# cheukwaylee/ORB_SLAM2_detailed_comments

Hardware: AMD Instinct MI355X
Metric: frames/sec ORB extract+match (1000 kp, 640x480) (higher is better)
Workload: dtype u8; 1 GPU; synthetic 640x480 mono stream, nFeatures=1000, 8 levels, scale 1.2, FAST 20/7, extract+match(t vs t-1), batch 1024 frames/GPU resident in HBM, 1 pipelines/GPU; parallelism=single GPU

## Files before the change

orb_slam2_detailed_comments_amd/csrc/orbx_api.cpp:

```cpp
#include <hip/hip_runtime.h>
#include <dlfcn.h>
#include <cstdio>
#include <cstdlib>
#include <cstring>
#include <string>
#include <vector>
#include <algorithm>
#include <cmath>
#include "orbx_internal.h"
#include "orbx_launch.h"
#include "orbx_gate.h"

static thread_local std::string g_last_error;
#define ORBX_RGBD_INPLACE_DEFAULT true

static orbx_status fail(orbx_status s, const std::string &msg) {
    g_last_error = msg;
    return s;
}
#define HIPCHK(expr)                                                                              \
    do {                                                                                          \
        hipError_t _e = (expr);                                                                   \
        if (_e != hipSuccess)                                                                     \
            return fail(ORBX_HIP_ERROR, std::string(#expr) + ": " + hipGetErrorString(_e));      \
// ... 13 lines not shown
    hipEvent_t ev_fork = nullptr, ev_join = nullptr;
    hipEvent_t ev_stereo = nullptr;
    int fork_level = 0;
    int fork_group = 0;
    int pipeline = 2;
    bool pipe_head = true;
    bool fast_room = false;
    hipEvent_t ev_pipe[ORBX_PIPE_MAX] = {};
    uint8_t *d_pyr = nullptr, *d_blur = nullptr;
    OrbxCell *d_cells = nullptr;
    OrbxFastGroup *d_groups = nullptr;
    bool resize_legacy = false;
    int match_kernel = 0;
    int fast_stop = 0;
    int fast_lcap = 640;
    OrbxTap *d_taps = nullptr;
    uint2 *d_dense = nullptr;
    int *d_cand_count = nullptr, *d_lvl_count = nullptr, *d_status = nullptr;
    uint32_t *d_lvl_kp = nullptr;
    float *d_lvl_angle = nullptr;
    uint16_t *d_knode = nullptr;
    int max_cw = 0, max_ch = 0, ncap = 0, lds_keys = 0, lds_keys_few = 0;
    uint8_t *st_in[2] = {nullptr, nullptr}; size_t d_in_bytes = 0;
    orbx_keypoint *st_kps[2] = {nullptr, nullptr}; uint8_t *st_desc[2] = {nullptr, nullptr}; int *st_cnt[2] = {nullptr, nullptr};
    int out_cap = 0, stage_chunk = 0;
    int *pin_stat = nullptr; size_t pin_stat_ints = 0;
    hipStream_t s_in = nullptr;
    hipEvent_t ev_in[2] = {nullptr, nullptr}, ev_done[2] = {nullptr, nullptr}, ev_out[2] = {nullptr, nullptr};
    uint8_t *st_dep[2] = {nullptr, nullptr}; size_t dep_bytes = 0;
    uint8_t *st_rg[2] = {nullptr, nullptr}; size_t rg_bytes = 0;
    int last_batch = 0;
// ... 87 lines not shown
    if (h->pending.empty()) return;
    hipStreamSynchronize(h->stream);
    for (auto &pp : h->pending) {
        float ms = 0;
        if (hipEventElapsedTime(&ms, pp.a, pp.b) == hipSuccess) { h->ms[pp.kid] += ms; h->launches[pp.kid]++; }
        h->pool.push_back(pp.a); h->pool.push_back(pp.b);
    }
    h->pending.clear();
}

static orbx_status pin_reserve(orbx_handle *h, size_t bytes);

static void free_geometry_buffers(orbx_handle *h) {
    hipFree(h->d_groups); h->d_groups = nullptr;
    hipFree(h->d_pyr); hipFree(h->d_blur); hipFree(h->d_cells); hipFree(h->d_taps);
    hipFree(h->d_dense); h->d_dense = nullptr;
    hipFree(h->d_cand_count); hipFree(h->d_lvl_count); hipFree(h->d_status); hipFree(h->d_lvl_kp);
    hipFree(h->d_lvl_angle); hipFree(h->d_knode);
    h->d_pyr = h->d_blur = nullptr; h->d_cells = nullptr; h->d_taps = nullptr;
    h->d_cand_count = h->d_lvl_count = h->d_status = nullptr; h->d_lvl_kp = nullptr; h->d_lvl_angle = nullptr;
    h->d_knode = nullptr;
    h->configured = false;
}

static orbx_status configure(orbx_handle *h, int width, int height) {
    if (h->configured && h->geom.width == width && h->geom.height == height) return ORBX_OK;
    if (h->host_only) return fail(ORBX_NO_DEVICE, "host-only handle (device = -2) cannot extract");
    HIPCHK(hipSetDevice(h->dev));
    if (h->configured) {
        HIPCHK(hipStreamSynchronize(h->stream));
// ... 40 lines not shown
            const size_t budget = (size_t)(160 * 1024) / wg - 512;
            return budget <= node_part ? 0 : std::min<size_t>({(budget - node_part) / 6, (size_t)4096, (size_t)g.max_cand_cap});
        };
        size_t keys_few = 0;
        for (int wg = 4; wg >= 2 && keys == 0; --wg)
            if (fit_at(wg) >= want) { keys = std::max<size_t>(want, 1024); keys_few = fit_at(wg); }
        h->lds_keys_few = (int)keys_few;
        if (keys == 0 && fit_at(2) >= 1024) keys = fit_at(2);
        if (keys == 0) keys = fit_at(1);
        if (const char *e = getenv("ORBX_QT_LDS_KEYS")) keys = std::min<size_t>((size_t)std::max(atoi(e), 0), std::min<size_t>(8192, (160 * 1024 - node_part) / 6));
        h->lds_keys = (int)keys;
        if (getenv("ORBX_QT_LDS_KEYS") || h->lds_keys_few < h->lds_keys) h->lds_keys_few = h->lds_keys;
    }
    HIPCHK(orbx_quadtree_prepare(orbx_quadtree_smem(h->ncap, std::max(h->lds_keys, h->lds_keys_few))));
    if (const char *e = getenv("ORBX_RESIZE_IMPL")) h->resize_legacy = strcmp(e, "legacy") == 0;
#ifdef ORBX_TIMING_KNOBS
    if (const char *e = getenv("ORBX_FAST_STOP")) h->fast_stop = atoi(e);
#endif
    if (const char *e = getenv("ORBX_FAST_LCAP")) h->fast_lcap = std::max(64, atoi(e));
    const OrbxGeom &hg = h->geom;
    hipStream_t s = h->stream;
    h->fork_level = 0;
    if (const char *e = getenv("ORBX_FORK_LEVEL")) h->fork_level = std::min(std::max(atoi(e), 0), NL - 1);
    h->fork_group = 0;
    if (h->fork_level > 0) {
        while (h->fork_group < (int)hg.fast_groups.size() && hg.cells[(size_t)hg.fast_groups[(size_t)h->fork_group].cell0].level < h->fork_level)
            ++h->fork_group;
        if (h->fork_group == 0 || h->fork_group >= (int)hg.fast_groups.size()) h->fork_level = 0;
    }
    if (const char *e = getenv("ORBX_PIPELINE")) h->pipeline = std::min(std::max(atoi(e), 0), ORBX_PIPE_MAX);
// ... 7 lines not shown
        ORBX_TRY(hipMalloc(&h->d_cells, std::max<size_t>(1, hg.cells.size()) * sizeof(OrbxCell)));
        ORBX_TRY(hipMalloc(&h->d_taps, std::max<size_t>(1, hg.taps.size()) * sizeof(OrbxTap)));
        ORBX_TRY(hipMalloc(&h->d_dense, (size_t)B * hg.cand_total * sizeof(uint2)));
        ORBX_TRY(hipMalloc(&h->d_knode, (size_t)B * hg.cand_total * sizeof(uint16_t)));
        ORBX_TRY(hipMalloc(&h->d_cand_count, (size_t)B * NL * sizeof(int)));
        ORBX_TRY(hipMalloc(&h->d_lvl_count, (size_t)B * NL * sizeof(int)));
        ORBX_TRY(hipMalloc(&h->d_status, (size_t)B * sizeof(int)));
        ORBX_TRY(hipMalloc(&h->d_lvl_kp, (size_t)B * hg.kp_total * sizeof(uint32_t)));
        ORBX_TRY(hipMalloc(&h->d_lvl_angle, (size_t)B * hg.kp_total * sizeof(float)));
        ORBX_TRY(hipMalloc(&h->d_groups, std::max<size_t>(1, hg.fast_groups.size()) * sizeof(OrbxFastGroup)));
        if (!hg.cells.empty()) {
            ORBX_TRY(hipMemcpyAsync(h->d_cells, hg.cells.data(), hg.cells.size() * sizeof(OrbxCell), hipMemcpyHostToDevice, s));
            ORBX_TRY(hipMemcpyAsync(h->d_groups, hg.fast_groups.data(), hg.fast_groups.size() * sizeof(OrbxFastGroup),
                                    hipMemcpyHostToDevice, s));
        }
        if (!hg.taps.empty())
            ORBX_TRY(hipMemcpyAsync(h->d_taps, hg.taps.data(), hg.taps.size() * sizeof(OrbxTap), hipMemcpyHostToDevice, s));
        ORBX_TRY(hipMemsetAsync(h->d_pyr, 0, (size_t)B * hg.pyr_bytes + 256, s));
        ORBX_TRY(hipMemsetAsync(h->d_lvl_count, 0, (size_t)B * NL * sizeof(int), s));
        ORBX_TRY(hipMemsetAsync(h->d_cand_count, 0, (size_t)B * NL * sizeof(int), s));
#undef ORBX_TRY
        return hipSuccess;
    };
    const hipError_t se = setup();
    if (se != hipSuccess) {
        hipStreamSynchronize(s);
        free_geometry_buffers(h);
        return fail(ORBX_HIP_ERROR, std::string("configure: ") + hipGetErrorString(se));
    }
    h->configured = true;
    h->last_batch = 0;
    return ORBX_OK;
// ... 143 lines not shown
    const DGeom &g = h->dg;
    hipStream_t s = h->stream;
    const int NL = g.nlevels;
    if (h->d_rect && (h->rect_w != W || h->rect_h != H))
        return fail(ORBX_BAD_ARGUMENT, "rectification maps were set for another image size (raw and rectified size must agree)");
    const int ngroups = (int)h->geom.fast_groups.size();
    auto pyramid = [&](hipStream_t st, int f0, int b, int l_end) {
        const uint8_t *im = d_imgs + (int64_t)f0 * frame_stride;
        uint8_t *pyr = h->d_pyr + (size_t)f0 * h->geom.pyr_bytes;
        int32_t *stp = d_status + f0;
        int *cc = h->d_cand_count + (size_t)f0 * NL;
        { ProfScope ps(h, ORBX_K_PYR_L0, st);
          if (h->d_rect) {
              orbx_launch_pyr_l0_remap(st, g, b, im, W, H, stride, frame_stride, pyr, h->d_rect, stp, cc);
          } else if (h->input_format == ORBX_FMT_GRAY8) {
              orbx_launch_pyr_l0(st, g, b, im, W, H, stride, frame_stride, pyr, stp, cc);
          } else {
              const int nch = (h->input_format == ORBX_FMT_RGB8 || h->input_format == ORBX_FMT_BGR8) ? 3 : 4;
              const bool rgb = h->input_format == ORBX_FMT_RGB8 || h->input_format == ORBX_FMT_RGBA8;
              orbx_launch_pyr_l0_color(st, g, b, im, W, H, stride, frame_stride, pyr, nch, rgb ? 0 : 2, rgb ? 2 : 0, stp, cc);
          } }
        for (int l = 1; l < l_end; ++l) {
            ProfScope ps(h, ORBX_K_PYR_RESIZE, st);
            orbx_launch_pyr_resize(st, g, b, l, h->d_taps, pyr, h->geom.lv[l].narrow_taps && !h->resize_legacy);
        }
    };
    auto fast = [&](hipStream_t st, int f0, int b, int g0, int ng, int lds_floor) {
        ProfScope ps(h, ORBX_K_FAST, st);
        orbx_launch_fast_rows(st, g, b, h->d_cells, h->d_groups + g0, ng, h->d_pyr + (size_t)f0 * h->geom.pyr_bytes,
                              h->d_dense + (size_t)f0 * g.cand_total, h->d_cand_count + (size_t)f0 * NL, d_status + f0, h->max_ch,
                              h->fast_lcap, h->fast_stop, lds_floor);
    };
    auto finish = [&](int f0, int b) {
        { ProfScope ps(h, ORBX_K_QUADTREE);
          orbx_launch_quadtree(s, g, b, h->d_dense + (size_t)f0 * g.cand_total, h->d_cand_count + (size_t)f0 * NL,
                               h->d_lvl_kp + (size_t)f0 * g.kp_total, h->d_lvl_count + (size_t)f0 * NL, d_status + f0,
                               h->d_knode + (size_t)f0 * g.cand_total, h->ncap, (long long)b * NL >= 1024 ? h->lds_keys : h->lds_keys_few, 0, NL); }
        { ProfScope ps(h, ORBX_K_DESC);
          orbx_launch_describe(s, g, b, h->d_pyr + (size_t)f0 * h->geom.pyr_bytes, h->d_lvl_kp + (size_t)f0 * g.kp_total,
// ... 27 lines not shown
            finish(off[k], off[k + 1] - off[k]);
        }
        hipError_t e = hipGetLastError();
        if (e != hipSuccess) { hipStreamSynchronize(s2); return fail(ORBX_HIP_ERROR, std::string("kernel launch: ") + hipGetErrorString(e)); }
        h->last_batch = B;
        return ORBX_OK;
    }
    const bool fork = h->fork_level > 0 && (long long)B * ngroups >= 16384;
    pyramid(s, 0, B, fork ? h->fork_level : NL);
    if (fork) {
        hipStream_t s2 = h->side_stream;
        if (hipEventRecord(h->ev_fork, s) != hipSuccess || hipStreamWaitEvent(s2, h->ev_fork, 0) != hipSuccess)
            return fail(ORBX_HIP_ERROR, "fork event");
        for (int l = h->fork_level; l < NL; ++l) {
            ProfScope ps(h, ORBX_K_PYR_RESIZE, s2);
            orbx_launch_pyr_resize(s2, g, B, l, h->d_taps, h->d_pyr, h->geom.lv[l].narrow_taps && !h->resize_legacy);
        }
        fast(s2, 0, B, h->fork_group, ngroups - h->fork_group, 0);
        fast(s, 0, B, 0, h->fork_group, 0);
        if (hipEventRecord(h->ev_join, s2) != hipSuccess || hipStreamWaitEvent(s, h->ev_join, 0) != hipSuccess)
            { hipStreamSynchronize(s2); return fail(ORBX_HIP_ERROR, "join event"); }
    } else {
        fast(s, 0, B, 0, ngroups, 0);
    }
    finish(0, B);
    hipError_t e = hipGetLastError();
    if (e != hipSuccess) return fail(ORBX_HIP_ERROR, std::string("kernel launch: ") + hipGetErrorString(e));
    h->last_batch = B;
    return ORBX_OK;
}

// ... 1464 lines not shown
```

orb_slam2_detailed_comments_amd/csrc/orbx_geometry.cpp:

```cpp
#include "orbx_internal.h"
#include <cmath>
#include <algorithm>

static inline int cv_round_f(float v) { return (int)lrintf(v); }
static inline int cv_round_d(double v) { return (int)lrint(v); }
static inline int cv_floor_f(float v) { int i = (int)v; return i - (i > v); }
static inline int cv_ceil_f(float v) { int i = (int)v; return i + (i < v); }
static inline int16_t sat16(int v) { return (int16_t)std::min(32767, std::max(-32768, v)); }
static inline int reflect101(int i, int n) {
    if (n == 1) return 0;
    while (i < 0 || i >= n) i = i < 0 ? -i : 2 * (n - 1) - i;
    return i;
}

void orbx_build_tables(const orbx_params &p, OrbxTables &t) {
    const int L = p.nlevels;
    const double sf = (double)p.scale_factor;
    t.scale[0] = 1.0f;
    t.sigma2[0] = 1.0f;
    for (int i = 1; i < L; ++i) {
        t.scale[i] = (float)((double)t.scale[i - 1] * sf);
        t.sigma2[i] = t.scale[i] * t.scale[i];
    }
    for (int i = 0; i < L; ++i) {
// ... 141 lines not shown
        }
    }
    for (size_t i = 0; i < g.cells.size();) {
        const OrbxCell &a = g.cells[i];
        OrbxFastGroup grp;
        grp.cell0 = (int32_t)i; grp.ncell = 1;
        if (i + 1 < g.cells.size()) {
            const OrbxCell &b = g.cells[i + 1];
            const bool adjacent = b.level == a.level && b.y0 == a.y0 && b.ch == a.ch && b.x0 == a.x0 + a.cw - 6 &&
                                  b.idx_in_level == a.idx_in_level + 1;
            if (adjacent && (a.cw - 6) + (b.cw - 6) <= 64 + ORBX_FAST_XCOLS) grp.ncell = 2;
        }
        g.fast_groups.push_back(grp);
        i += (size_t)grp.ncell;
    }
    g.pyr_bytes = off;
    g.cand_total = cand_off;
    g.kp_total = kp_off;
    return ORBX_OK;
}
```

orb_slam2_detailed_comments_amd/csrc/orbx_internal.h:

```cpp
#pragma once
#include <cstdint>
#include <vector>
#include "../../include/orbx.h"

#define ORBX_MAX_LEVELS 16
#define ORBX_EDGE 19
#define ORBX_HALF_PATCH 15
#define ORBX_PATCH 31
#define ORBX_NPATCH 749

struct OrbxCell {
    int16_t x0, y0, cw, ch;
    int16_t offx, offy;
    int16_t level;
    int16_t idx_in_level;
    int32_t slot_begin;
    int32_t slot_cap;
};

#define ORBX_FAST_XCOLS 2
struct OrbxFastGroup {
    int32_t cell0;
    int32_t ncell;
};
#define ORBX_LDS_PER_CU (160 * 1024)
#define ORBX_FAST_PIPE_WAVES 16
#define ORBX_PIPE_MAX 8
#define ORBX_PIPE_MIN_FRAMES 256

struct OrbxTap {
    int16_t s0, s1;
    int16_t a0, a1;
};

struct OrbxLevelGeom {
    int sw, sh;
    int pw, ph, pitch;
    int64_t off;
    int ncols, nrows, wcell, hcell;
    int cell_begin, cell_count;
    int qt_w, qt_h;
    int nini;
    float hx;
    int nfeat;
    int kp_cap;
    int kp_begin;
    int cand_cap;
    int64_t cand_begin;
    int tapx_begin, tapy_begin;
    bool narrow_taps;
    float scale;
    float size;
};

struct OrbxGeom {
    int width = 0, height = 0, nlevels = 0;
    OrbxLevelGeom lv[ORBX_MAX_LEVELS];
    std::vector<OrbxCell> cells;
    std::vector<OrbxFastGroup> fast_groups;
    std::vector<OrbxTap> taps;
    int64_t pyr_bytes = 0;
    int64_t cand_total = 0;
    int kp_total = 0;
    int node_cap = 0;
    int max_cand_cap = 0;
};

struct OrbxTables {
    float scale[ORBX_MAX_LEVELS], inv_scale[ORBX_MAX_LEVELS], sigma2[ORBX_MAX_LEVELS], inv_sigma2[ORBX_MAX_LEVELS];
    int nfeat[ORBX_MAX_LEVELS];
    int umax[ORBX_HALF_PATCH + 1];
};

void orbx_build_tables(const orbx_params &p, OrbxTables &t);
orbx_status orbx_build_geometry(const orbx_params &p, const OrbxTables &t, int width, int height, OrbxGeom &g,
// ... 2 lines not shown
```

orb_slam2_detailed_comments_amd/csrc/orbx_kernels.hip:

```cpp
#include "orbx_device.h"
#include "../../include/orbx_pattern_data.h"

#define L0_ROWS 8
#ifndef L0_FF
#define L0_FF 1
#endif
#ifndef RR_FF
#define RR_FF 1
#endif
#ifndef QT_FF
#define QT_FF 1
#endif
__global__ __launch_bounds__(256) void k_pyr_l0(DGeom g, const uint8_t *__restrict__ imgs, int W, int H, int stride,
                                                long long frame_stride, uint8_t *__restrict__ pyr, int xe,
                                                int *__restrict__ status, int *__restrict__ cand_cursor) {
    const DLevel &L = g.lv[0];
#if L0_FF
    const int f = blockIdx.x, bx = blockIdx.y, by = blockIdx.z, nbx = gridDim.y;
#else
    const int f = blockIdx.z, bx = blockIdx.x, by = blockIdx.y, nbx = gridDim.x;
#endif
    if (bx == 0 && by == 0 && threadIdx.y == 0) {
        if (threadIdx.x == 0) status[f] = 0;
        if ((int)threadIdx.x < g.nlevels) cand_cursor[f * g.nlevels + threadIdx.x] = 0;
// ... 26 lines not shown
#pragma unroll
        for (int r = 0; r < L0_ROWS; ++r) {
            const int Y = Y0 + r;
            if (Y >= L.ph) break;
            const uint8_t *src = img + (long long)orbx_reflect101(Y - ORBX_EDGE, H) * stride;
            uint32_t w = 0;
#pragma unroll
            for (int i = 0; i < 4; ++i) {
                const int x = X + i;
                const uint32_t p = x < L.pw ? src[orbx_reflect101(x - ORBX_EDGE, W)] : 0u;
                w |= p << (8 * i);
            }
            *(uint32_t *)(dst + (long long)Y * L.pitch + X) = w;
        }
    }
}

__global__ __launch_bounds__(256) void k_pyr_l0_color(DGeom g, const uint8_t *__restrict__ imgs, int W, int H, int stride,
                                                      long long frame_stride, uint8_t *__restrict__ pyr, int nch,
                                                      int r_off, int b_off, int *__restrict__ status, int *__restrict__ cand_cursor) {
    const DLevel &L = g.lv[0];
    const int X = (blockIdx.x * 64 + threadIdx.x) * 4;
    const int Y = blockIdx.y * 4 + threadIdx.y;
    const int f = blockIdx.z;
    if (blockIdx.x == 0 && blockIdx.y == 0 && threadIdx.y == 0) {
        if (threadIdx.x == 0) status[f] = 0;
        if ((int)threadIdx.x < g.nlevels) cand_cursor[f * g.nlevels + threadIdx.x] = 0;
    }
    if (X >= L.pw || Y >= L.ph) return;
    const uint8_t *src = imgs + (long long)f * frame_stride + (long long)orbx_reflect101(Y - ORBX_EDGE, H) * stride;
// ... 39 lines not shown
            const uint8_t *r0 = src + (long long)iy * stride + ix, *r1 = r0 + stride;
            const uint32_t p00 = (x0 && y0) ? r0[0] : 0u, p01 = (x1 && y0) ? r0[1] : 0u, p10 = (x0 && y1) ? r1[0] : 0u,
                           p11 = (x1 && y1) ? r1[1] : 0u;
            const uint32_t acc = __umul24((32u - fx) * (32u - fy) * 32u, p00) + __umul24(fx * (32u - fy) * 32u, p01) +
                                 __umul24((32u - fx) * fy * 32u, p10) + __umul24(fx * fy * 32u, p11);
            p = (acc + (1u << 14)) >> 15;
        }
        v |= p << (8 * i);
    }
    *(uint32_t *)(pyr + (long long)f * g.pyr_bytes + L.off + (long long)Y * L.pitch + X) = v;
}

struct __attribute__((packed, aligned(1))) orbx_uint2_u { uint32_t x, y; };
struct __attribute__((packed, aligned(1))) orbx_uint3_u { uint32_t x, y, z; };
__device__ __forceinline__ uint2 orbx_load8(const void *p) { const orbx_uint2_u v = *(const orbx_uint2_u *)p; return make_uint2(v.x, v.y); }
struct __attribute__((aligned(4))) orbx_uint3_a { uint32_t x, y, z; };
typedef unsigned short orbx_v2u16 __attribute__((ext_vector_type(2)));
__device__ __forceinline__ uint32_t orbx_udot2(uint32_t a, uint32_t b) {
    return __builtin_amdgcn_udot2(__builtin_bit_cast(orbx_v2u16, a), __builtin_bit_cast(orbx_v2u16, b), 0u, false);
}
#define RS_ROWS 2
__global__ __launch_bounds__(256) void k_pyr_resize(DGeom g, int level, const OrbxTap *__restrict__ taps,
                                                    uint8_t *__restrict__ pyr) {
    const DLevel &L = g.lv[level];
    const DLevel &S = g.lv[level - 1];
    const int X = (blockIdx.x * 64 + threadIdx.x) * 4;
    const int Y0 = (blockIdx.y * 4 + threadIdx.y) * RS_ROWS;
    const int f = blockIdx.z;
    if (X >= L.pw || Y0 >= L.ph) return;
    uint8_t *base = pyr + (long long)f * g.pyr_bytes;
    OrbxTap tx[4];
    int smin = 0x7fff, smax = 0;
#pragma unroll
    for (int i = 0; i < 4; ++i) {
// ... 75 lines not shown
                const int T1 = r1[tx[i].s0] * tx[i].a0 + r1[tx[i].s1] * tx[i].a1;
                const uint32_t p = (uint32_t)((((((b0 & 0xfff) * ((T0 >> 4) & 0xffff))) >> 16) + ((((b1 & 0xfff) * ((T1 >> 4) & 0xffff))) >> 16) + 2) >> 2) & 0xffu;
                v |= p << (8 * i);
            }
        }
        *(uint32_t *)(base + L.off + (long long)Y * L.pitch + X) = v;
    }
}

#ifndef RR_REVERSE
#define RR_REVERSE 1
#endif
#ifndef RR_WPB
#define RR_WPB 1
#endif
__global__ __launch_bounds__(64 * RR_WPB) void k_pyr_resize_rows(DGeom g, int level, const OrbxTap *__restrict__ taps,
                                                         uint8_t *__restrict__ pyr, int rpw) {
    const DLevel &L = g.lv[level];
    const DLevel &S = g.lv[level - 1];
    const int lane = threadIdx.x;
#if RR_FF
    const int f = blockIdx.x, bx = blockIdx.y;
    const int by = (RR_REVERSE && (level & 1)) ? (int)gridDim.z - 1 - (int)blockIdx.z : (int)blockIdx.z;
#else
    const int f = blockIdx.z, bx = blockIdx.x, by = blockIdx.y;
#endif
    const int X = (bx * 64 + lane) * 4;
    const int y_begin = __builtin_amdgcn_readfirstlane((by * RR_WPB + threadIdx.y) * rpw);
    if (y_begin >= L.ph) return;
    const int y_end = min(y_begin + rpw, L.ph);
    const bool on = X < L.pw;
    uint8_t *base = pyr + (long long)f * g.pyr_bytes;
// ... 6 lines not shown
        const uint2 *tq = (const uint2 *)taps + L.tapx;
        uint2 t[4];
#pragma unroll
        for (int i = 0; i < 4; ++i) t[i] = tq[min(X + i, L.pw - 1)];
#pragma unroll
        for (int i = 0; i < 4; ++i) smin = min(smin, (int)(t[i].x & 0xffffu));
#pragma unroll
        for (int i = 0; i < 4; ++i) {
            const uint32_t d = (t[i].x & 0xffffu) - (uint32_t)smin;
            sel[i] = d | (0x0cu << 8) | ((d + 1u) << 16) | (0x0cu << 24);
            wgt[i] = t[i].y;
        }
    }
    const uint32_t sh = (uint32_t)(smin & 3);
    const uint32_t lsrc = (uint32_t)(smin & ~3);
    const uint2 *ty = (const uint2 *)taps + L.tapy;
#ifndef RR_R
#define RR_R 2
#endif
#define RR_H(dst, v)                                                                                                     \
    {                                                                                                                   \
        const uint32_t lo_ = __builtin_amdgcn_alignbyte((v).y, (v).x, sh), hi_ = __builtin_amdgcn_alignbyte((v).z, (v).y, sh); \
        _Pragma("unroll") for (int i = 0; i < 4; ++i)                                                                   \
            dst[i] = orbx_udot2(__builtin_amdgcn_perm(hi_, lo_, sel[i]), wgt[i]) >> 4;                                  \
    }
#define RR_V(out, h0, h1, w0, w1)                                                                                       \
    {                                                                                                                   \
        out = 0;                                                                                                        \
        _Pragma("unroll") for (int i = 0; i < 4; ++i)                                                                   \
            out |= (((__umul24(w0, h0[i]) >> 16) + (__umul24(w1, h1[i]) >> 16) + 2u) >> 2) << (8 * i);                  \
    }
    uint2 t[RR_R];
    orbx_uint3_a u[RR_R], w[RR_R];
    int pid = -1;
    uint32_t hb[2][4] = {{0, 0, 0, 0}, {0, 0, 0, 0}};
#pragma unroll
    for (int r = 0; r < RR_R; ++r) {
        t[r] = ty[min(y_begin + r, L.ph - 1)];
        u[r].x = u[r].y = u[r].z = 0;
        if (r == 0 || (int)(t[r].x & 0xffffu) != (int)(t[r - 1].x >> 16)) u[r] = *(const orbx_uint3_a *)(src + (uint32_t)((t[r].x & 0xffffu) * (uint32_t)S.pitch + lsrc));
        w[r] = *(const orbx_uint3_a *)(src + (uint32_t)((t[r].x >> 16) * (uint32_t)S.pitch + lsrc));
    }
    for (int Y = y_begin; Y < y_end; Y += RR_R) {
        uint2 ct[RR_R];
        orbx_uint3_a cu[RR_R], cw[RR_R];
#pragma unroll
        for (int r = 0; r < RR_R; ++r) { ct[r] = t[r]; cu[r] = u[r]; cw[r] = w[r]; }
        if (Y + RR_R < y_end) {
            int last = (int)(ct[RR_R - 1].x >> 16);
#pragma unroll
            for (int r = 0; r < RR_R; ++r) {
                t[r] = ty[min(Y + RR_R + r, L.ph - 1)];
                const int s0 = (int)(t[r].x & 0xffffu), s1 = (int)(t[r].x >> 16);
                if (s0 != last) u[r] = *(const orbx_uint3_a *)(src + (uint32_t)((uint32_t)s0 * (uint32_t)S.pitch + lsrc));
                w[r] = *(const orbx_uint3_a *)(src + (uint32_t)((uint32_t)s1 * (uint32_t)S.pitch + lsrc));
                last = s1;
            }
        }
#pragma unroll
        for (int r = 0; r < RR_R; ++r) {
            uint32_t (&h0)[4] = hb[r & 1], (&h1)[4] = hb[(r & 1) ^ 1];
            const int s0 = (int)(ct[r].x & 0xffffu);
            if (s0 != pid) RR_H(h0, cu[r])
            RR_H(h1, cw[r])
            uint32_t v;
            RR_V(v, h0, h1, ct[r].y & 0xfffu, (ct[r].y >> 16) & 0xfffu)
            pid = (int)(ct[r].x >> 16);
            if (on && Y + r < y_end) *(uint32_t *)(dst + (uint32_t)((uint32_t)(Y + r) * (uint32_t)L.pitch + ldst)) = v;
        }
    }
#undef RR_H
#undef RR_V
}

__device__ __forceinline__ bool orbx_arc9(uint32_t mask16) {
    uint32_t m = mask16 | (mask16 << 16);
    uint32_t a = m & (m >> 1);
    a &= a >> 2;
    a &= a >> 4;
    a &= m >> 8;
    return (a & 0xffffu) != 0;
}

__device__ __forceinline__ unsigned long long orbx_ballot(bool p) { return __builtin_amdgcn_ballot_w64(p); }
__device__ __forceinline__ int orbx_wave_rank(unsigned long long bal) {
// ... 2413 lines not shown
            for (int sl = 0; sl < 16; ++sl) {
                const int k = 16 * (lane >> 4) + sl, i = k - (16 * j + (lane & 15));
                if (i >= 0 && i <= 6) bb[j][lane][sl >> 2] |= (uint32_t)K7[i] << (8 * (sl & 3));
            }
    return hipMemcpyToSymbol(HIP_SYMBOL(c_blur_b), bb, sizeof(bb));
}

size_t orbx_quadtree_smem(int ncap, int lds_keys) {
    return 128 + (size_t)ncap * (8 * 4 + 16 + 8 + 6 * 4) + 16 + (size_t)lds_keys * 6 + 16;
}

void orbx_launch_clear(hipStream_t s, int *a, int na, int *b, int nb, int *c, int nc) {
    const int n = na > nb ? (na > nc ? na : nc) : (nb > nc ? nb : nc);
    hipLaunchKernelGGL(k_clear, dim3((n + 255) / 256), dim3(256), 0, s, a, na, b, nb, c, nc);
}
void orbx_launch_pyr_l0(hipStream_t s, const DGeom &g, int B, const uint8_t *imgs, int W, int H, int stride,
                        long long frame_stride, uint8_t *pyr, int *status, int *cand_cursor) {
    const DLevel &L = g.lv[0];
    int xe = 32;
    while (xe + 1 <= W) xe += 16;
    const int icols = (xe - 32 + 1023) / 1024;
#if L0_FF
    dim3 grid(B, icols + 1, (L.ph + 4 * L0_ROWS - 1) / (4 * L0_ROWS));
#else
    dim3 grid(icols + 1, (L.ph + 4 * L0_ROWS - 1) / (4 * L0_ROWS), B);
#endif
    hipLaunchKernelGGL(k_pyr_l0, grid, dim3(64, 4), 0, s, g, imgs, W, H, stride, frame_stride, pyr, xe, status, cand_cursor);
}
void orbx_launch_pyr_l0_color(hipStream_t s, const DGeom &g, int B, const uint8_t *imgs, int W, int H, int stride,
                              long long frame_stride, uint8_t *pyr, int nch, int r_off, int b_off, int *status, int *cand_cursor) {
    const DLevel &L = g.lv[0];
    dim3 grid((L.pw + 255) / 256, (L.ph + 3) / 4, B);
    hipLaunchKernelGGL(k_pyr_l0_color, grid, dim3(64, 4), 0, s, g, imgs, W, H, stride, frame_stride, pyr, nch, r_off, b_off, status, cand_cursor);
}
void orbx_launch_pyr_l0_remap(hipStream_t s, const DGeom &g, int B, const uint8_t *imgs, int W, int H, int stride,
                              long long frame_stride, uint8_t *pyr, const uint2 *rect, int *status, int *cand_cursor) {
    const DLevel &L = g.lv[0];
    dim3 grid((L.pw + 255) / 256, (L.ph + 3) / 4, B);
    hipLaunchKernelGGL(k_pyr_l0_remap, grid, dim3(64, 4), 0, s, g, imgs, W, H, stride, frame_stride, pyr, rect, status, cand_cursor);
}
void orbx_launch_pyr_resize(hipStream_t s, const DGeom &g, int B, int level, const OrbxTap *taps, uint8_t *pyr, bool narrow) {
    const DLevel &L = g.lv[level];
    if (narrow) {
        int rpw = 16;
        while (rpw > 2 && (long long)((L.pw + 255) / 256) * ((L.ph + rpw - 1) / rpw) * B < 4096) rpw >>= 1;
#if RR_FF
        dim3 grid(B, (L.pw + 255) / 256, (L.ph + RR_WPB * rpw - 1) / (RR_WPB * rpw));
#else
        dim3 grid((L.pw + 255) / 256, (L.ph + RR_WPB * rpw - 1) / (RR_WPB * rpw), B);
#endif
        hipLaunchKernelGGL(k_pyr_resize_rows, grid, dim3(64, RR_WPB), 0, s, g, level, taps, pyr, rpw);
        return;
    }
    dim3 grid((L.pw + 255) / 256, (L.ph + 4 * RS_ROWS - 1) / (4 * RS_ROWS), B);
    hipLaunchKernelGGL(k_pyr_resize, grid, dim3(64, 4), 0, s, g, level, taps, pyr);
}
void orbx_launch_fast_rows(hipStream_t s, const DGeom &g, int B, const OrbxCell *cells, const OrbxFastGroup *groups,
                           int ngroups, const uint8_t *pyr, uint2 *cand, int *cand_cursor, int *status, int max_ch, int lcap,
                           int dbg_stop, int lds_floor) {
    if (ngroups <= 0) return;
    lcap = (max(lcap, 64) + 1) & ~1;
    const int ccap = min(lcap, FR_CCAP);
    const size_t map_bytes = ((size_t)max_ch * FR_TP + 15) & ~(size_t)15;
    const size_t need = 2 * map_bytes + (size_t)2 * lcap + 256 + (size_t)2 * ccap;
    const size_t smem = lds_floor > 0 && (size_t)lds_floor > need ? (size_t)lds_floor : need;
    const int gpw = (long long)B * ngroups >= 16384 ? FR_GPW : 1;
// ... 219 lines not shown
```

orb_slam2_detailed_comments_amd/csrc/orbx_launch.h:

```cpp
#pragma once
#include <hip/hip_runtime.h>
#include "orbx_device.h"

hipError_t orbx_upload_pattern();
size_t orbx_quadtree_smem(int ncap, int lds_keys);
hipError_t orbx_quadtree_prepare(size_t smem);
void orbx_launch_clear(hipStream_t s, int *a, int na, int *b, int nb, int *c, int nc);
void orbx_launch_pyr_l0(hipStream_t s, const DGeom &g, int B, const uint8_t *imgs, int W, int H, int stride,
                        long long frame_stride, uint8_t *pyr, int *status, int *cand_cursor);
void orbx_launch_pyr_l0_color(hipStream_t s, const DGeom &g, int B, const uint8_t *imgs, int W, int H, int stride,
                              long long frame_stride, uint8_t *pyr, int nch, int r_off, int b_off, int *status, int *cand_cursor);
void orbx_launch_pyr_l0_remap(hipStream_t s, const DGeom &g, int B, const uint8_t *imgs, int W, int H, int stride,
                              long long frame_stride, uint8_t *pyr, const uint2 *rect, int *status, int *cand_cursor);
void orbx_launch_pyr_resize(hipStream_t s, const DGeom &g, int B, int level, const OrbxTap *taps, uint8_t *pyr, bool narrow);
void orbx_launch_fast_rows(hipStream_t s, const DGeom &g, int B, const OrbxCell *cells, const OrbxFastGroup *groups,
                           int ngroups, const uint8_t *pyr, uint2 *cand, int *cand_cursor, int *status, int max_ch, int lcap,
                           int dbg_stop, int lds_floor = 0);
void orbx_launch_undistort(hipStream_t s, int B, int max_n, int cap, const double *K4, const double *k14, int identity,
                           const orbx_keypoint *kps, const int *counts, orbx_keypoint *out);
struct OrbxRgbdArgs {
    const uint8_t *depth; long long frame_stride, stride;
    int format, width, height, scale_f32;
    float scale, mbf;
};
void orbx_launch_rgbd(hipStream_t s, int B, int max_n, int cap, const double *K4, const double *k14, int identity,
                      const OrbxRgbdArgs &a, const orbx_keypoint *kps, const orbx_keypoint *kun_in, const int *counts,
                      orbx_keypoint *kun_out, float *u_right, float *depth);
void orbx_launch_bow_transform(hipStream_t s, int B, int max_n, const int *child_begin, const uint32_t *child_ids,
                               const uint8_t *node_desc, int n_nodes, int L, const uint8_t *desc, const int *counts,
// ... 42 lines not shown
```

Measured before the change: 334,200 frames/s.

## Add chunked level-0 pyramid copy with seam tables and precomputed resize row steps

Replaces the grayscale level-0 border-copy kernel with a flat 1D-chunked kernel. Interior 16-byte chunks are built from aligned dword loads plus alignbyte, and border chunks use a host-precomputed seam table with byte permutes for reflect101 padding. The row-resize kernel now reads precomputed row offsets and weights, ping-pongs two prefetch buffers, and uses v_mul_hi_u32_u24 for the vertical weighting. The aim is less address arithmetic and better load/compute overlap in pyramid construction, at the cost of extra device tables and more complex indexing code.

```diff
diff --git a/orb_slam2_detailed_comments_amd/csrc/orbx_api.cpp b/orb_slam2_detailed_comments_amd/csrc/orbx_api.cpp
--- a/orb_slam2_detailed_comments_amd/csrc/orbx_api.cpp
+++ b/orb_slam2_detailed_comments_amd/csrc/orbx_api.cpp
@@ -51,7 +51,10 @@
     int match_kernel = 0;
     int fast_stop = 0;
     int fast_lcap = 640;
+    bool l0_legacy = false;
     OrbxTap *d_taps = nullptr;
+    OrbxL0Seam *d_l0_seams = nullptr;
+    OrbxRowStep *d_row_steps = nullptr;
     uint2 *d_dense = nullptr;
     int *d_cand_count = nullptr, *d_lvl_count = nullptr, *d_status = nullptr;
     uint32_t *d_lvl_kp = nullptr;
@@ -169,6 +172,7 @@
 static void free_geometry_buffers(orbx_handle *h) {
     hipFree(h->d_groups); h->d_groups = nullptr;
     hipFree(h->d_pyr); hipFree(h->d_blur); hipFree(h->d_cells); hipFree(h->d_taps);
+    hipFree(h->d_l0_seams); hipFree(h->d_row_steps); h->d_l0_seams = nullptr; h->d_row_steps = nullptr;
     hipFree(h->d_dense); h->d_dense = nullptr;
     hipFree(h->d_cand_count); hipFree(h->d_lvl_count); hipFree(h->d_status); hipFree(h->d_lvl_kp);
     hipFree(h->d_lvl_angle); hipFree(h->d_knode);
@@ -239,6 +243,7 @@
     }
     HIPCHK(orbx_quadtree_prepare(orbx_quadtree_smem(h->ncap, std::max(h->lds_keys, h->lds_keys_few))));
     if (const char *e = getenv("ORBX_RESIZE_IMPL")) h->resize_legacy = strcmp(e, "legacy") == 0;
+    if (const char *e = getenv("ORBX_L0_IMPL")) h->l0_legacy = strcmp(e, "legacy") == 0;
 #ifdef ORBX_TIMING_KNOBS
     if (const char *e = getenv("ORBX_FAST_STOP")) h->fast_stop = atoi(e);
 #endif
@@ -276,8 +281,15 @@
             ORBX_TRY(hipMemcpyAsync(h->d_groups, hg.fast_groups.data(), hg.fast_groups.size() * sizeof(OrbxFastGroup),
                                     hipMemcpyHostToDevice, s));
         }
-        if (!hg.taps.empty())
+        if (!hg.taps.empty()) {
             ORBX_TRY(hipMemcpyAsync(h->d_taps, hg.taps.data(), hg.taps.size() * sizeof(OrbxTap), hipMemcpyHostToDevice, s));
+            ORBX_TRY(hipMalloc(&h->d_row_steps, hg.row_steps.size() * sizeof(OrbxRowStep)));
+            ORBX_TRY(hipMemcpyAsync(h->d_row_steps, hg.row_steps.data(), hg.row_steps.size() * sizeof(OrbxRowStep), hipMemcpyHostToDevice, s));
+        }
+        if (!hg.l0_seams.empty()) {
+            ORBX_TRY(hipMalloc(&h->d_l0_seams, hg.l0_seams.size() * sizeof(OrbxL0Seam)));
+            ORBX_TRY(hipMemcpyAsync(h->d_l0_seams, hg.l0_seams.data(), hg.l0_seams.size() * sizeof(OrbxL0Seam), hipMemcpyHostToDevice, s));
+        }
         ORBX_TRY(hipMemsetAsync(h->d_pyr, 0, (size_t)B * hg.pyr_bytes + 256, s));
         ORBX_TRY(hipMemsetAsync(h->d_lvl_count, 0, (size_t)B * NL * sizeof(int), s));
         ORBX_TRY(hipMemsetAsync(h->d_cand_count, 0, (size_t)B * NL * sizeof(int), s));
@@ -451,7 +463,7 @@
           if (h->d_rect) {
               orbx_launch_pyr_l0_remap(st, g, b, im, W, H, stride, frame_stride, pyr, h->d_rect, stp, cc);
           } else if (h->input_format == ORBX_FMT_GRAY8) {
-              orbx_launch_pyr_l0(st, g, b, im, W, H, stride, frame_stride, pyr, stp, cc);
+              orbx_launch_pyr_l0(st, g, b, im, W, H, stride, frame_stride, pyr, stp, cc, h->l0_legacy ? nullptr : h->d_l0_seams);
           } else {
               const int nch = (h->input_format == ORBX_FMT_RGB8 || h->input_format == ORBX_FMT_BGR8) ? 3 : 4;
               const bool rgb = h->input_format == ORBX_FMT_RGB8 || h->input_format == ORBX_FMT_RGBA8;
@@ -459,7 +471,7 @@
           } }
         for (int l = 1; l < l_end; ++l) {
             ProfScope ps(h, ORBX_K_PYR_RESIZE, st);
-            orbx_launch_pyr_resize(st, g, b, l, h->d_taps, pyr, h->geom.lv[l].narrow_taps && !h->resize_legacy);
+            orbx_launch_pyr_resize(st, g, b, l, h->d_taps, pyr, h->geom.lv[l].narrow_taps && !h->resize_legacy, h->d_row_steps);
         }
     };
     auto fast = [&](hipStream_t st, int f0, int b, int g0, int ng, int lds_floor) {
@@ -517,7 +529,7 @@
             return fail(ORBX_HIP_ERROR, "fork event");
         for (int l = h->fork_level; l < NL; ++l) {
             ProfScope ps(h, ORBX_K_PYR_RESIZE, s2);
-            orbx_launch_pyr_resize(s2, g, B, l, h->d_taps, h->d_pyr, h->geom.lv[l].narrow_taps && !h->resize_legacy);
+            orbx_launch_pyr_resize(s2, g, B, l, h->d_taps, h->d_pyr, h->geom.lv[l].narrow_taps && !h->resize_legacy, h->d_row_steps);
         }
         fast(s2, 0, B, h->fork_group, ngroups - h->fork_group, 0);
         fast(s, 0, B, 0, h->fork_group, 0);
diff --git a/orb_slam2_detailed_comments_amd/csrc/orbx_geometry.cpp b/orb_slam2_detailed_comments_amd/csrc/orbx_geometry.cpp
--- a/orb_slam2_detailed_comments_amd/csrc/orbx_geometry.cpp
+++ b/orb_slam2_detailed_comments_amd/csrc/orbx_geometry.cpp
@@ -179,6 +179,41 @@
         g.fast_groups.push_back(grp);
         i += (size_t)grp.ncell;
     }
+    g.row_steps.assign(g.taps.size(), OrbxRowStep{0, 0, 0, 0});
+    for (int l = 1; l < p.nlevels; ++l) {
+        const OrbxLevelGeom &L = g.lv[l], &S = g.lv[l - 1];
+        for (int Y = 0; Y < L.ph; ++Y) {
+            const OrbxTap &ty = g.taps[(size_t)L.tapy_begin + Y];
+            OrbxRowStep &rs = g.row_steps[(size_t)L.tapy_begin + Y];
+            rs.off0 = (uint32_t)ty.s0 * (uint32_t)S.pitch;
+            rs.off1 = (uint32_t)ty.s1 * (uint32_t)S.pitch;
+            rs.w0 = ((uint32_t)ty.a0 & 0xfffu) << 12;
+            rs.w1 = ((uint32_t)ty.a1 & 0xfffu) << 12;
+        }
+    }
+    if (width >= ORBX_L0_MIN_W && height > ORBX_EDGE) {
+        const OrbxLevelGeom &L = g.lv[0];
+        for (int X = 0; X < L.pitch; X += 16) {
+            OrbxL0Seam c;
+            for (int k = 0; k < 4; ++k) {
+                int sidx[4], lo = 0x7fffffff, hi = -1;
+                for (int i = 0; i < 4; ++i) {
+                    const int x = X + 4 * k + i;
+                    sidx[i] = x < L.pw ? reflect101(x - ORBX_EDGE, width) : -1;
+                    if (sidx[i] >= 0) { lo = std::min(lo, sidx[i]); hi = std::max(hi, sidx[i]); }
+                }
+                c.r[k] = 0; c.sel[k] = 0; c.keep[k] = 0;
+                if (hi < 0) continue;
+                c.r[k] = hi < width / 2 ? lo : hi - 4;
+                for (int i = 0; i < 4; ++i)
+                    if (sidx[i] >= 0) {
+                        c.sel[k] |= (uint32_t)(sidx[i] - c.r[k]) << (8 * i);
+                        c.keep[k] |= 0xffu << (8 * i);
+                    }
+            }
+            g.l0_seams.push_back(c);
+        }
+    }
     g.pyr_bytes = off;
     g.cand_total = cand_off;
     g.kp_total = kp_off;
diff --git a/orb_slam2_detailed_comments_amd/csrc/orbx_internal.h b/orb_slam2_detailed_comments_amd/csrc/orbx_internal.h
--- a/orb_slam2_detailed_comments_amd/csrc/orbx_internal.h
+++ b/orb_slam2_detailed_comments_amd/csrc/orbx_internal.h
@@ -33,6 +33,16 @@
     int16_t a0, a1;
 };
 
+#define ORBX_L0_MIN_W 96
+struct OrbxL0Seam {
+    int32_t r[4];
+    uint32_t sel[4];
+    uint32_t keep[4];
+};
+struct OrbxRowStep {
+    uint32_t off0, off1, w0, w1;
+};
+
 struct OrbxLevelGeom {
     int sw, sh;
     int pw, ph, pitch;
@@ -59,6 +69,8 @@
     std::vector<OrbxCell> cells;
     std::vector<OrbxFastGroup> fast_groups;
     std::vector<OrbxTap> taps;
+    std::vector<OrbxL0Seam> l0_seams;
+    std::vector<OrbxRowStep> row_steps;
     int64_t pyr_bytes = 0;
     int64_t cand_total = 0;
     int kp_total = 0;
diff --git a/orb_slam2_detailed_comments_amd/csrc/orbx_kernels.hip b/orb_slam2_detailed_comments_amd/csrc/orbx_kernels.hip
--- a/orb_slam2_detailed_comments_amd/csrc/orbx_kernels.hip
+++ b/orb_slam2_detailed_comments_amd/csrc/orbx_kernels.hip
@@ -64,6 +64,68 @@
             *(uint32_t *)(dst + (long long)Y * L.pitch + X) = w;
         }
     }
+}
+
+__global__ __launch_bounds__(256) void k_pyr_l0_chunks(DGeom g, const uint8_t *__restrict__ imgs, int W, int H, int stride,
+                                                       long long frame_stride, uint8_t *__restrict__ pyr,
+                                                       const OrbxL0Seam *__restrict__ seams, int nch, uint32_t nch_magic,
+                                                       int nitems, int *__restrict__ status, int *__restrict__ cand_cursor) {
+    const DLevel &L = g.lv[0];
+    const int f = blockIdx.x;
+    if (blockIdx.y == 0) {
+        if (threadIdx.x == 0) status[f] = 0;
+        if ((int)threadIdx.x < g.nlevels) cand_cursor[f * g.nlevels + threadIdx.x] = 0;
+    }
+    const uint32_t item = blockIdx.y * 256u + threadIdx.x;
+    if (item >= (uint32_t)nitems) return;
+    const uint32_t band = __umulhi(item, nch_magic);
+    const int X = (int)(item - band * (uint32_t)nch) * 16;
+    const int Y0 = (int)band * L0_ROWS;
+    const uint8_t *img = imgs + (long long)f * frame_stride;
+    const uint32_t a0 = (uint32_t)((unsigned long long)img & 3ull);
+    const uint8_t *base = img - a0;
+    uint8_t *dst = pyr + (long long)f * g.pyr_bytes + L.off;
+    uint32_t ro[L0_ROWS];
+#pragma unroll
+    for (int r = 0; r < L0_ROWS; ++r) {
+        int t = min(Y0 + r, L.ph - 1) - ORBX_EDGE;
+        t = max(t, -t);
+        t = min(t, 2 * (H - 1) - t);
+        ro[r] = (uint32_t)t * (uint32_t)stride + a0;
+    }
+    uint4 v[L0_ROWS];
+    if (X >= 32 && X <= W + 2) {
+#pragma unroll
+        for (int r = 0; r < L0_ROWS; ++r) {
+            const uint32_t o = ro[r] + (uint32_t)(X - ORBX_EDGE);
+            const uint32_t m = o & 3u;
+            const uint32_t *ap = (const uint32_t *)(base + (o & ~3u));
+            const uint32_t q0 = ap[0], q1 = ap[1], q2 = ap[2], q3 = ap[3], q4 = ap[4];
+            v[r] = make_uint4(__builtin_amdgcn_alignbyte(q1, q0, m), __builtin_amdgcn_alignbyte(q2, q1, m),
+                              __builtin_amdgcn_alignbyte(q3, q2, m), __builtin_amdgcn_alignbyte(q4, q3, m));
+        }
+    } else {
+        const uint4 *sp = (const uint4 *)(seams + (X >> 4));
+        const uint4 sr = sp[0], ss = sp[1], sk = sp[2];
+        const uint32_t rr[4] = {sr.x, sr.y, sr.z, sr.w}, sel[4] = {ss.x, ss.y, ss.z, ss.w}, keep[4] = {sk.x, sk.y, sk.z, sk.w};
+#pragma unroll
+        for (int r = 0; r < L0_ROWS; ++r) {
+            uint32_t d[4];
+#pragma unroll
+            for (int k = 0; k < 4; ++k) {
+                const uint32_t o = ro[r] + rr[k];
+                const uint32_t m = o & 3u;
+                const uint32_t *ap = (const uint32_t *)(base + (o & ~3u));
+                const uint32_t lo = ap[0], hi = ap[1];
+                const uint32_t m4 = __builtin_amdgcn_perm(0u, m, 0u);
+                d[k] = __builtin_amdgcn_perm(hi, lo, sel[k] + m4) & keep[k];
+            }
+            v[r] = make_uint4(d[0], d[1], d[2], d[3]);
+        }
+    }
+#pragma unroll
+    for (int r = 0; r < L0_ROWS; ++r)
+        *(uint4 *)(dst + __umul24((uint32_t)min(Y0 + r, L.ph - 1), (uint32_t)L.pitch) + (uint32_t)X) = v[r];
 }
 
 __global__ __launch_bounds__(256) void k_pyr_l0_color(DGeom g, const uint8_t *__restrict__ imgs, int W, int H, int stride,
@@ -133,10 +195,15 @@
 struct __attribute__((packed, aligned(1))) orbx_uint2_u { uint32_t x, y; };
 struct __attribute__((packed, aligned(1))) orbx_uint3_u { uint32_t x, y, z; };
 __device__ __forceinline__ uint2 orbx_load8(const void *p) { const orbx_uint2_u v = *(const orbx_uint2_u *)p; return make_uint2(v.x, v.y); }
-struct __attribute__((aligned(4))) orbx_uint3_a { uint32_t x, y, z; };
+typedef uint32_t orbx_v3u_a __attribute__((ext_vector_type(3), aligned(4)));
 typedef unsigned short orbx_v2u16 __attribute__((ext_vector_type(2)));
 __device__ __forceinline__ uint32_t orbx_udot2(uint32_t a, uint32_t b) {
     return __builtin_amdgcn_udot2(__builtin_bit_cast(orbx_v2u16, a), __builtin_bit_cast(orbx_v2u16, b), 0u, false);
+}
+__device__ __forceinline__ uint32_t orbx_mulhi_u24(uint32_t a, uint32_t b) {
+    uint32_t d;
+    asm("v_mul_hi_u32_u24 %0, %1, %2" : "=v"(d) : "s"(a), "v"(b));
+    return d;
 }
 #define RS_ROWS 2
 __global__ __launch_bounds__(256) void k_pyr_resize(DGeom g, int level, const OrbxTap *__restrict__ taps,
@@ -242,8 +309,11 @@
 #ifndef RR_WPB
 #define RR_WPB 1
 #endif
+#ifndef RR_MULHI
+#define RR_MULHI 1
+#endif
 __global__ __launch_bounds__(64 * RR_WPB) void k_pyr_resize_rows(DGeom g, int level, const OrbxTap *__restrict__ taps,
-                                                         uint8_t *__restrict__ pyr, int rpw) {
+                                                         const OrbxRowStep *__restrict__ steps, uint8_t *__restrict__ pyr, int rpw) {
     const DLevel &L = g.lv[level];
     const DLevel &S = g.lv[level - 1];
     const int lane = threadIdx.x;
@@ -280,61 +350,73 @@
     }
     const uint32_t sh = (uint32_t)(smin & 3);
     const uint32_t lsrc = (uint32_t)(smin & ~3);
-    const uint2 *ty = (const uint2 *)taps + L.tapy;
+    const uint4 *ts = (const uint4 *)steps + L.tapy;
 #ifndef RR_R
 #define RR_R 2
+#endif
+#if RR_MULHI
+#define RR_HFIX(x) ((x) & ~15u)
+#define RR_VMUL(wgt, h) orbx_mulhi_u24(wgt, h)
+#else
+#define RR_HFIX(x) ((x) >> 4)
+#define RR_VMUL(wgt, h) (__umul24((wgt) >> 12, h) >> 16)
 #endif
 #define RR_H(dst, v)                                                                                                     \
     {                                                                                                                   \
         const uint32_t lo_ = __builtin_amdgcn_alignbyte((v).y, (v).x, sh), hi_ = __builtin_amdgcn_alignbyte((v).z, (v).y, sh); \
         _Pragma("unroll") for (int i = 0; i < 4; ++i)                                                                   \
-            dst[i] = orbx_udot2(__builtin_amdgcn_perm(hi_, lo_, sel[i]), wgt[i]) >> 4;                                  \
+            dst[i] = RR_HFIX(orbx_udot2(__builtin_amdgcn_perm(hi_, lo_, sel[i]), wgt[i]));                              \
     }
 #define RR_V(out, h0, h1, w0, w1)                                                                                       \
     {                                                                                                                   \
         out = 0;                                                                                                        \
         _Pragma("unroll") for (int i = 0; i < 4; ++i)                                                                   \
-            out |= (((__umul24(w0, h0[i]) >> 16) + (__umul24(w1, h1[i]) >> 16) + 2u) >> 2) << (8 * i);                  \
-    }
-    uint2 t[RR_R];
-    orbx_uint3_a u[RR_R], w[RR_R];
-    int pid = -1;
+            out |= ((RR_VMUL(w0, h0[i]) + RR_VMUL(w1, h1[i]) + 2u) >> 2) << (8 * i);                                    \
+    }
+#define RR_FETCH(T, U, W, YN, LAST)                                                                                      \
+    {                                                                                                                   \
+        uint32_t last_ = (LAST);                                                                                        \
+        _Pragma("unroll") for (int r = 0; r < RR_R; ++r) {                                                              \
+            T[r] = ts[min((YN) + r, L.ph - 1)];                                                                         \
+            if (T[r].x != last_) U[r] = *(const orbx_v3u_a *)(src + (uint32_t)(T[r].x + lsrc));                         \
+            W[r] = *(const orbx_v3u_a *)(src + (uint32_t)(T[r].y + lsrc));                                              \
+            last_ = T[r].y;                                                                                             \
+        }                                                                                                               \
+    }
+#define RR_EVAL(T, U, W, YY)                                                                                             \
+    {                                                                                                                   \
+        _Pragma("unroll") for (int r = 0; r < RR_R; ++r) {                                                              \
+            uint32_t (&h0)[4] = hb[r & 1], (&h1)[4] = hb[(r & 1) ^ 1];                                                  \
+            if (T[r].x != pid) RR_H(h0, U[r])                                                                           \
+            RR_H(h1, W[r])                                                                                              \
+            uint32_t v;                                                                                                 \
+            RR_V(v, h0, h1, T[r].z, T[r].w)                                                                             \
+            pid = T[r].y;                                                                                               \
+            if (on && (YY) + r < y_end) *(uint32_t *)(dst + odst) = v;                                                  \
+            odst += (uint32_t)L.pitch;                                                                                  \
+        }                                                                                                               \
+    }
+    uint4 tA[RR_R], tB[RR_R];
+    orbx_v3u_a uA[RR_R], wA[RR_R], uB[RR_R], wB[RR_R];
+#pragma unroll
+    for (int r = 0; r < RR_R; ++r) uA[r] = uB[r] = orbx_v3u_a{0, 0, 0};
+    uint32_t pid = 0xffffffffu;
     uint32_t hb[2][4] = {{0, 0, 0, 0}, {0, 0, 0, 0}};
-#pragma unroll
-    for (int r = 0; r < RR_R; ++r) {
-        t[r] = ty[min(y_begin + r, L.ph - 1)];
-        u[r].x = u[r].y = u[r].z = 0;
-        if (r == 0 || (int)(t[r].x & 0xffffu) != (int)(t[r - 1].x >> 16)) u[r] = *(const orbx_uint3_a *)(src + (uint32_t)((t[r].x & 0xffffu) * (uint32_t)S.pitch + lsrc));
-        w[r] = *(const orbx_uint3_a *)(src + (uint32_t)((t[r].x >> 16) * (uint32_t)S.pitch + lsrc));
-    }
-    for (int Y = y_begin; Y < y_end; Y += RR_R) {
-        uint2 ct[RR_R];
-        orbx_uint3_a cu[RR_R], cw[RR_R];
-#pragma unroll
-        for (int r = 0; r < RR_R; ++r) { ct[r] = t[r]; cu[r] = u[r]; cw[r] = w[r]; }
-        if (Y + RR_R < y_end) {
-            int last = (int)(ct[RR_R - 1].x >> 16);
-#pragma unroll
-            for (int r = 0; r < RR_R; ++r) {
-                t[r] = ty[min(Y + RR_R + r, L.ph - 1)];
-                const int s0 = (int)(t[r].x & 0xffffu), s1 = (int)(t[r].x >> 16);
-                if (s0 != last) u[r] = *(const orbx_uint3_a *)(src + (uint32_t)((uint32_t)s0 * (uint32_t)S.pitch + lsrc));
-                w[r] = *(const orbx_uint3_a *)(src + (uint32_t)((uint32_t)s1 * (uint32_t)S.pitch + lsrc));
-                last = s1;
-            }
-        }
-#pragma unroll
-        for (int r = 0; r < RR_R; ++r) {
-            uint32_t (&h0)[4] = hb[r & 1], (&h1)[4] = hb[(r & 1) ^ 1];
-            const int s0 = (int)(ct[r].x & 0xffffu);
-            if (s0 != pid) RR_H(h0, cu[r])
-            RR_H(h1, cw[r])
-            uint32_t v;
-            RR_V(v, h0, h1, ct[r].y & 0xfffu, (ct[r].y >> 16) & 0xfffu)
-            pid = (int)(ct[r].x >> 16);
-            if (on && Y + r < y_end) *(uint32_t *)(dst + (uint32_t)((uint32_t)(Y + r) * (uint32_t)L.pitch + ldst)) = v;
-        }
-    }
+    uint32_t odst = (uint32_t)y_begin * (uint32_t)L.pitch + ldst;
+    RR_FETCH(tA, uA, wA, y_begin, 0xffffffffu)
+    for (int Y = y_begin; Y < y_end; Y += 2 * RR_R) {
+        const bool more = Y + RR_R < y_end;
+        if (more) RR_FETCH(tB, uB, wB, Y + RR_R, tA[RR_R - 1].y)
+        RR_EVAL(tA, uA, wA, Y)
+        if (more) {
+            if (Y + 2 * RR_R < y_end) RR_FETCH(tA, uA, wA, Y + 2 * RR_R, tB[RR_R - 1].y)
+            RR_EVAL(tB, uB, wB, Y + RR_R)
+        }
+    }
+#undef RR_FETCH
+#undef RR_EVAL
+#undef RR_HFIX
+#undef RR_VMUL
 #undef RR_H
 #undef RR_V
 }
@@ -2778,8 +2860,8 @@
     const int n = na > nb ? (na > nc ? na : nc) : (nb > nc ? nb : nc);
     hipLaunchKernelGGL(k_clear, dim3((n + 255) / 256), dim3(256), 0, s, a, na, b, nb, c, nc);
 }
-void orbx_launch_pyr_l0(hipStream_t s, const DGeom &g, int B, const uint8_t *imgs, int W, int H, int stride,
-                        long long frame_stride, uint8_t *pyr, int *status, int *cand_cursor) {
+static void orbx_launch_pyr_l0_legacy(hipStream_t s, const DGeom &g, int B, const uint8_t *imgs, int W, int H, int stride,
+                                      long long frame_stride, uint8_t *pyr, int *status, int *cand_cursor) {
     const DLevel &L = g.lv[0];
     int xe = 32;
     while (xe + 1 <= W) xe += 16;
@@ -2791,6 +2873,18 @@
 #endif
     hipLaunchKernelGGL(k_pyr_l0, grid, dim3(64, 4), 0, s, g, imgs, W, H, stride, frame_stride, pyr, xe, status, cand_cursor);
 }
+void orbx_launch_pyr_l0(hipStream_t s, const DGeom &g, int B, const uint8_t *imgs, int W, int H, int stride,
+                        long long frame_stride, uint8_t *pyr, int *status, int *cand_cursor, const OrbxL0Seam *seams) {
+    const DLevel &L = g.lv[0];
+    if (!seams || W < ORBX_L0_MIN_W || H <= ORBX_EDGE || (long long)H * stride + 8 >= (1ll << 31)) {
+        orbx_launch_pyr_l0_legacy(s, g, B, imgs, W, H, stride, frame_stride, pyr, status, cand_cursor);
+        return;
+    }
+    const int nch = L.pitch / 16, nitems = nch * ((L.ph + L0_ROWS - 1) / L0_ROWS);
+    const uint32_t magic = (uint32_t)((1ull << 32) / (unsigned)nch + 1);
+    hipLaunchKernelGGL(k_pyr_l0_chunks, dim3(B, (nitems + 255) / 256), dim3(256), 0, s, g, imgs, W, H, stride, frame_stride, pyr,
+                       seams, nch, magic, nitems, status, cand_cursor);
+}
 void orbx_launch_pyr_l0_color(hipStream_t s, const DGeom &g, int B, const uint8_t *imgs, int W, int H, int stride,
                               long long frame_stride, uint8_t *pyr, int nch, int r_off, int b_off, int *status, int *cand_cursor) {
     const DLevel &L = g.lv[0];
@@ -2803,9 +2897,10 @@
     dim3 grid((L.pw + 255) / 256, (L.ph + 3) / 4, B);
     hipLaunchKernelGGL(k_pyr_l0_remap, grid, dim3(64, 4), 0, s, g, imgs, W, H, stride, frame_stride, pyr, rect, status, cand_cursor);
 }
-void orbx_launch_pyr_resize(hipStream_t s, const DGeom &g, int B, int level, const OrbxTap *taps, uint8_t *pyr, bool narrow) {
+void orbx_launch_pyr_resize(hipStream_t s, const DGeom &g, int B, int level, const OrbxTap *taps, uint8_t *pyr, bool narrow,
+                            const OrbxRowStep *steps) {
     const DLevel &L = g.lv[level];
-    if (narrow) {
+    if (narrow && steps) {
         int rpw = 16;
         while (rpw > 2 && (long long)((L.pw + 255) / 256) * ((L.ph + rpw - 1) / rpw) * B < 4096) rpw >>= 1;
 #if RR_FF
@@ -2813,7 +2908,7 @@
 #else
         dim3 grid((L.pw + 255) / 256, (L.ph + RR_WPB * rpw - 1) / (RR_WPB * rpw), B);
 #endif
-        hipLaunchKernelGGL(k_pyr_resize_rows, grid, dim3(64, RR_WPB), 0, s, g, level, taps, pyr, rpw);
+        hipLaunchKernelGGL(k_pyr_resize_rows, grid, dim3(64, RR_WPB), 0, s, g, level, taps, steps, pyr, rpw);
         return;
     }
     dim3 grid((L.pw + 255) / 256, (L.ph + 4 * RS_ROWS - 1) / (4 * RS_ROWS), B);
diff --git a/orb_slam2_detailed_comments_amd/csrc/orbx_launch.h b/orb_slam2_detailed_comments_amd/csrc/orbx_launch.h
--- a/orb_slam2_detailed_comments_amd/csrc/orbx_launch.h
+++ b/orb_slam2_detailed_comments_amd/csrc/orbx_launch.h
@@ -7,12 +7,14 @@
 hipError_t orbx_quadtree_prepare(size_t smem);
 void orbx_launch_clear(hipStream_t s, int *a, int na, int *b, int nb, int *c, int nc);
 void orbx_launch_pyr_l0(hipStream_t s, const DGeom &g, int B, const uint8_t *imgs, int W, int H, int stride,
-                        long long frame_stride, uint8_t *pyr, int *status, int *cand_cursor);
+                        long long frame_stride, uint8_t *pyr, int *status, int *cand_cursor,
+                        const OrbxL0Seam *seams = nullptr);
 void orbx_launch_pyr_l0_color(hipStream_t s, const DGeom &g, int B, const uint8_t *imgs, int W, int H, int stride,
                               long long frame_stride, uint8_t *pyr, int nch, int r_off, int b_off, int *status, int *cand_cursor);
 void orbx_launch_pyr_l0_remap(hipStream_t s, const DGeom &g, int B, const uint8_t *imgs, int W, int H, int stride,
                               long long frame_stride, uint8_t *pyr, const uint2 *rect, int *status, int *cand_cursor);
-void orbx_launch_pyr_resize(hipStream_t s, const DGeom &g, int B, int level, const OrbxTap *taps, uint8_t *pyr, bool narrow);
+void orbx_launch_pyr_resize(hipStream_t s, const DGeom &g, int B, int level, const OrbxTap *taps, uint8_t *pyr, bool narrow,
+                            const OrbxRowStep *steps = nullptr);
 void orbx_launch_fast_rows(hipStream_t s, const DGeom &g, int B, const OrbxCell *cells, const OrbxFastGroup *groups,
                            int ngroups, const uint8_t *pyr, uint2 *cand, int *cand_cursor, int *status, int max_ch, int lcap,
                            int dbg_stop, int lds_floor = 0);
```

After: 339,800 frames/s (median of 6 runs). +1.7%, better.
